# zhangmozhe/Deep-Exemplar-based-Video-Colorization

Hardware: AMD Instinct MI355X
Metric: colorized frames/sec/GPU at 216x384; correlation HBM GB/s vs roofline (higher is better)
Workload: dtype f32

## Files before the change

deep-exemplar-based-video-colorization_amd/csrc/conv_mfma.hip:

```cpp
#include "conv_kernel.h"
#include "conv_sk_kernel.h"
#include <algorithm>

#include "conv_wino_kernel.h"

static int virt_dim(int S, int up, int sub) {
    if (up == 2) return S * 2;
    if (sub == 2) return (S + 1) / 2;
    return S;
}

extern "C" int dvc_conv2d_out_hw(const DvcConvDesc* d, int32_t* OH, int32_t* OW) {
    DVC_REQUIRE(d, "dvc_conv2d_out_hw: null descriptor");
    int VH = virt_dim(d->H, d->in_up, d->in_sub), VW = virt_dim(d->W, d->in_up, d->in_sub);
    int ext = d->dil * (d->ksize - 1) + 1;
    *OH = (VH + 2 * d->pad - ext) / d->stride + 1;
    *OW = (VW + 2 * d->pad - ext) / d->stride + 1;
    return 0;
}

static int pick_tw(int OW) {
    int best = 32, best_w = cdiv(OW, 32) * 32;
    for (int tw : {16, 8}) {
        int wpad = cdiv(OW, tw) * tw;
// ... 575 lines not shown
    s.m_cls = wino_magic((long)s.blk_y * s.blk_x);
    s.m_blkx = wino_magic(s.blk_x);
    s.m_split = wino_magic(s.k.split);
    return dim3((unsigned)(s.gx * s.gy * s.gz));
}

static int wino_reduce(const DvcConvDesc* d, const ConvWinoArgs& s, int NB, int OH, int OW, const float* bias,
                       const float* act_slope_ptr, hipStream_t st) {
    const ConvKArgs& a = s.k;
    const long OHW = (long)OH * OW, per_img = (long)d->Cout * OHW;
    if (a.split > 1 && s.pool) {
        const long windows = (long)d->Cout * ((OH + 1) / 2) * ((OW + 1) / 2);
        hipLaunchKernelGGL(conv_splitk_reduce_pool_kernel, dim3((unsigned)((windows + 255) / 256), NB), dim3(256), 0, st, a.part,
                           a.split, (long)NB * per_img, d->Cout, OH, OW, bias, d->act, d->act_slope, act_slope_ptr, a.y, a.y_bs,
                           s.pool, s.pool_bs);
        DVC_CHECK_LAUNCH("dvc_conv2d_winograd_pool(split-K reduce)");
    } else if (a.split > 1 && !(d->flags & DVC_CONV_DEFER_REDUCE)) {
        const bool v4 = (OHW % 4 == 0) && ((reinterpret_cast<uintptr_t>(a.part) & 15) == 0) && (((long)NB * per_img) % 4 == 0);
        if (v4)
            hipLaunchKernelGGL(conv_splitk_reduce_kernel<4>, dim3((unsigned)((per_img / 4 + 255) / 256), NB), dim3(256), 0, st,
                               a.part, a.split, (long)NB * per_img, d->Cout, OHW, bias, a.res, a.res_bs, d->act,
                               d->act_slope, act_slope_ptr, a.y, a.y_bs);
        else
            hipLaunchKernelGGL(conv_splitk_reduce_kernel<1>, dim3((unsigned)((per_img + 255) / 256), NB), dim3(256), 0, st,
                               a.part, a.split, (long)NB * per_img, d->Cout, OHW, bias, a.res, a.res_bs, d->act,
                               d->act_slope, act_slope_ptr, a.y, a.y_bs);
        DVC_CHECK_LAUNCH("dvc_conv2d_winograd(split-K reduce)");
    }
    return 0;
}

static int wino_run(const DvcConvDesc* d, const DvcConvDesc* d2, const float* x, const float* x2, const float* u_packed,
                    const float* bias, const float* act_slope_ptr, const float* residual, float* y, void* workspace,
                    size_t workspace_bytes, dvcStream stream, float* pool = nullptr, long pool_batch_stride = 0) {
    ConvWinoArgs s;
    int best_m = -1, best_tr = 1, group = 0;
    if (int rc = wino_setup(d, d2, x, x2, u_packed, bias, act_slope_ptr, residual, y, workspace, workspace_bytes, pool,
                            pool_batch_stride, s, &best_m, &best_tr, &group))
        return rc;
    ConvKArgs& a = s.k;
    int32_t OH, OW;
    dvc_conv2d_out_hw(d, &OH, &OW);
    hipStream_t st = (hipStream_t)stream;
    for (int n0 = 0; n0 < d->N; n0 += group) {
        const int NB = std::min(group, d->N - n0);
        a.N = NB;
        a.x = x + (long)n0 * a.x_bs;
        if (d2) s.x2 = x2 + (long)n0 * s.x2_bs;
        a.y = y ? y + (long)n0 * a.y_bs : nullptr;
        s.pool = pool ? pool + (long)n0 * s.pool_bs : nullptr;
        a.res = residual ? residual + (long)n0 * a.res_bs : nullptr;
        DVC_REQUIRE((long)s.gx * s.gy * NB * a.split < (1L << 31), "dvc_conv2d_winograd: grid too large");
        const dim3 grid = wino_finish_grid(s, NB);
        if (d2) conv_wino_launch_m1_dual(best_tr, grid, st, s);
        else if (best_m == 0) conv_wino_launch_m4(best_tr, grid, st, s);
        else if (best_m == 1) conv_wino_launch_m2(best_tr, grid, st, s);
        else if (best_m == 2) conv_wino_launch_m1(best_tr, grid, st, s);
        else conv_wino_launch_m0(best_tr, grid, st, s);
        DVC_CHECK_LAUNCH("dvc_conv2d_winograd");
        if (int rc = wino_reduce(d, s, NB, OH, OW, bias, act_slope_ptr, st)) return rc;
    }
    return 0;
}

extern "C" int dvc_conv2d_winograd_group(const DvcConvGroupItem* items, int32_t n_items, dvcStream stream) {
    DVC_REQUIRE(items && n_items >= 1 && n_items <= WINO_GROUP_MAX, "dvc_conv2d_winograd_group: 1..%d items", WINO_GROUP_MAX);
    hipStream_t st = (hipStream_t)stream;
    ConvWinoGroupArgs g;
    int OHs[WINO_GROUP_MAX], OWs[WINO_GROUP_MAX], order[WINO_GROUP_MAX];
    ConvWinoArgs tmp[WINO_GROUP_MAX];
    int trs[WINO_GROUP_MAX];
    bool together = n_items > 1;
    for (int i = 0; i < n_items; ++i) {
        const DvcConvGroupItem& it = items[i];
        DVC_REQUIRE(it.x && it.u_packed && it.y, "dvc_conv2d_winograd_group: null argument in item %d", i);
        for (int j = 0; j < i; ++j) DVC_REQUIRE(it.y != items[j].y, "dvc_conv2d_winograd_group: items %d and %d share an output", j, i);
        int m = -1, grp = 0;
        if (int rc = wino_setup(&it.d, nullptr, it.x, nullptr, it.u_packed, it.bias, it.act_slope_ptr, it.residual, it.y, it.workspace,
                                it.workspace_bytes, nullptr, 0, tmp[i], &m, &trs[i], &grp))
            return rc;
        int32_t oh, ow;
        dvc_conv2d_out_hw(&it.d, &oh, &ow);
        OHs[i] = oh; OWs[i] = ow;
        if (m != 2 || grp < it.d.N) together = false;
        for (int j = 0; j < i; ++j)
            DVC_REQUIRE(!(tmp[i].k.split > 1 && tmp[j].k.split > 1 && tmp[i].k.part == tmp[j].k.part),
                        "dvc_conv2d_winograd_group: the split items %d and %d share a workspace", j, i);
        order[i] = i;
    }
    if (!together) {
        for (int i = 0; i < n_items; ++i) {
            const DvcConvGroupItem& it = items[i];
            if (int rc = wino_run(&it.d, nullptr, it.x, nullptr, it.u_packed, it.bias, it.act_slope_ptr, it.residual, it.y, it.workspace,
                                  it.workspace_bytes, stream))
                return rc;
        }
        return 0;
    }
    std::sort(order, order + n_items, [&](int a, int b) {
        return tmp[a].k.chunks_per_split != tmp[b].k.chunks_per_split ? tmp[a].k.chunks_per_split > tmp[b].k.chunks_per_split : a < b;
    });
    g.n = n_items;
    g.per_xcd[0] = 0;
    for (int k = 0; k < WINO_GROUP_MAX; ++k) {
        const int i = order[k < n_items ? k : n_items - 1];
        g.item[k] = tmp[i];
        g.tr[k] = trs[i];
// ... 95 lines not shown
```

deep-exemplar-based-video-colorization_amd/csrc/conv_wino_kernel.h:

```cpp
#pragma once
#include <type_traits>

#include "conv_kernel.h"

typedef float f32x4 __attribute__((ext_vector_type(4)));
typedef float f32x2 __attribute__((ext_vector_type(2)));

struct ConvWinoArgs {
    ConvKArgs k;
    int ss;
    int blk_y, blk_x;
    int gx, gy, gz;
    unsigned m_gx, m_gxy, m_cls, m_blkx, m_split;
    const float* x2;
    long x2_bs;
    int cinA, H2, W2, VH2, VW2, in_up2, in_sub2;
    float* pool;
    long pool_bs;
};
__host__ __device__ __forceinline__ unsigned wino_magic(long d) {
    return d > 1 ? (unsigned)(((1ULL << 32) + (unsigned long long)d - 1) / (unsigned long long)d) : 0u;
}
__device__ __forceinline__ int wino_div(int n, unsigned magic) { return magic ? (int)__umulhi((unsigned)n, magic) : n; }

__host__ __device__ constexpr int wino_pitch(int tr) { return tr == 1 ? 66 : tr == 2 ? 48 : tr == 4 ? 24 : 12; }

#define WINO_A10(p) "a" #p "0", "a" #p "1", "a" #p "2", "a" #p "3", "a" #p "4", "a" #p "5", "a" #p "6", "a" #p "7", "a" #p "8", "a" #p "9"
#define WINO_AGPRS                                                                                                     \
    WINO_A10(), WINO_A10(1), WINO_A10(2), WINO_A10(3), WINO_A10(4), WINO_A10(5), WINO_A10(6), WINO_A10(7), WINO_A10(8), \
        WINO_A10(9), WINO_A10(10), WINO_A10(11), "a120", "a121", "a122", "a123", "a124", "a125", "a126", "a127"
#define WINO_MFMA(K, A, B)                                                                \
    asm volatile("s_nop 1\n\tv_mfma_f32_32x32x2_f32 a[%2:%3], %0, %1, a[%2:%3]"            \
                 :                                                                         \
                 : "v"(A), "v"(B), "i"((K) * 16), "i"((K) * 16 + 15)                       \
                 : WINO_AGPRS)
#define WINO_PK_ADD(D, A, B) asm volatile("v_pk_add_f32 %0, %1, %2" : "=v"(D) : "v"(A), "v"(B))
#define WINO_PK_SUB(D, A, B) asm volatile("v_pk_add_f32 %0, %1, %2 neg_lo:[0,1] neg_hi:[0,1]" : "=v"(D) : "v"(A), "v"(B))
#define WINO_PK_MID(D, A, B) \
    asm volatile("v_pk_add_f32 %0, %1, %2 op_sel:[0,1] op_sel_hi:[0,1] neg_hi:[0,1]" : "=v"(D) : "v"(A), "v"(B))

#define WINO_LOADS(D, U, XA, UA, UOFS)                                                                                 \
    asm volatile("ds_read2_b64 %0, %5 offset0:%7 offset1:%8\n\t"                                                        \
                 "ds_read2_b64 %1, %5 offset0:%9 offset1:%10\n\t"                                                       \
                 "ds_read2_b64 %2, %5 offset0:%11 offset1:%12\n\t"                                                      \
                 "ds_read_b128 %3, %6 offset:%13\n\t"                                                                   \
                 "ds_read_b128 %4, %6 offset:%14"                                                                       \
                 : "=&v"(D[0]), "=&v"(D[1]), "=&v"(D[2]), "=&v"(U[0]), "=&v"(U[1])                                      \
                 : "v"(XA), "v"(UA), "i"(0 * (PITCH / 2)), "i"(0 * (PITCH / 2) + 1), "i"(1 * (PITCH / 2)),              \
                   "i"(1 * (PITCH / 2) + 1), "i"(2 * (PITCH / 2)), "i"(2 * (PITCH / 2) + 1), "i"((UOFS) + 0),           \
                   "i"((UOFS) + 512)                                                                                    \
                 : "memory")
#define WINO_WAIT_LOADS(D, U)                                                                 \
    asm volatile("s_waitcnt lgkmcnt(0)"                                                        \
                 : "+v"(D[0]), "+v"(D[1]), "+v"(D[2]), "+v"(U[0]), "+v"(U[1])                  \
                 :                                                                             \
                 : "memory")

#define WINO_S_ADD(D, A, B) asm volatile("v_add_f32 %0, %1, %2" : "=v"(D) : "v"(A), "v"(B))
#define WINO_S_SUB(D, A, B) asm volatile("v_sub_f32 %0, %1, %2" : "=v"(D) : "v"(A), "v"(B))

__device__ __forceinline__ int wino_stored_offset(int VH, int VW, int W, int in_up, int in_sub, int pad_mode, int vy, int vx) {
    int sy = map_virtual(vy, VH, pad_mode);
    int sx = map_virtual(vx, VW, pad_mode);
    if (sy < 0 || sx < 0) return -1;
    if (in_up == 2) {
        sy >>= 1;
        sx >>= 1;
    } else if (in_sub == 2) {
        sy <<= 1;
        sx <<= 1;
    }
    return sy * W + sx;
}

#define WINO_NBUF 3
__host__ __device__ constexpr int wino_xs_floats(int wm, int wn, int tr, int kc) {
    return ((kc * (2 * tr * wn + 2) * wino_pitch(tr) + 128 * wm * wn - 1) / (128 * wm * wn)) * (128 * wm * wn);
}
__host__ __device__ constexpr int wino_us_floats(int wm, int kc) { return wm * kc * 128 * 4; }

template <int WM, int WN, int TR, int KC, int VAR = 0, bool DUAL = false, class SA = ConvWinoArgs>
__device__ __forceinline__ void conv_wino_body(const SA& s, const int wlog, float* const xsb, float* const usb) {
#if defined(__HIP_DEVICE_COMPILE__)
    const auto& a = s.k;
    constexpr int NPAIR = WM * WN;
    constexpr int NT = 128 * NPAIR;
    constexpr int TC = 32 / TR;
    constexpr int PR = 2 * TR * WN + 2;
    constexpr int PC = 2 * TC + 2;
    constexpr int PITCH = wino_pitch(TR);
    constexpr int plane = PR * PITCH;
    constexpr int EPT = (KC * plane + NT - 1) / NT;
    constexpr int C_XS = EPT * NT;
    static_assert(C_XS == wino_xs_floats(WM, WN, TR, KC), "LDS size helper out of step");
    constexpr int UQ = WM * KC * 128;
    static_assert(UQ * 4 == wino_us_floats(WM, KC), "LDS size helper out of step");
    static_assert(UQ % NT == 0, "whole staging instructions");
    static_assert(PITCH >= PC && PITCH % 2 == 0 && plane % 2 == 0 && KC % 4 == 0, "aligned patch rows, even K-steps per chunk");
    static_assert(2 * (PITCH / 2) + 1 < 256, "ds_read2_b64 offsets are 8 bits");
    constexpr int WPT = UQ / NT;
    constexpr int NI = EPT + WPT;
    static_assert(2 * NI < 64, "vmcnt is 6 bits");
    constexpr int KS = KC / 2;
    constexpr int NBUF = WINO_NBUF;
    constexpr int OOB = (int)0x80000000;
    static_assert(NBUF * UQ * 4 >= 2 * NPAIR * 32 * 64, "the output exchange fits in the filter buffers");

    const int tid = threadIdx.x;
    const int lane = tid & 63, wave = __builtin_amdgcn_readfirstlane(tid >> 6);
    const int l31 = lane & 31, hi = lane >> 5;
    const int ph = wave / NPAIR, pair = wave % NPAIR;
    const int wm = pair / WN, wn = pair % WN;
    const int tr = l31 / TC, tc = l31 % TC;
    const int ss = s.ss;
    const int bz = wino_div(wlog, s.m_gxy), r_xy = wlog - bz * (s.gx * s.gy);
    const int by = wino_div(r_xy, s.m_gx), bx = r_xy - by * s.gx;
    const int per_cls = s.blk_y * s.blk_x;
    const int cls = wino_div(bx, s.m_cls), brem = bx - cls * per_cls;
    const int py = ss == 2 ? cls >> 1 : 0, px = ss == 2 ? cls & 1 : 0;
    const int tyb = wino_div(brem, s.m_blkx);
    const int ty0 = tyb * (TR * WN), tx0 = (brem - tyb * s.blk_x) * TC;
    const int b0 = by * WM;
    const int n = wino_div(bz, s.m_split), ksplit = bz - n * a.split;
    const int HWi = a.H * a.W;

    const int nchunks_all = a.Cin / KC;
    const int c_begin = ksplit * a.chunks_per_split;
    const int c_end = min(nchunks_all, c_begin + a.chunks_per_split);

    int gofs[EPT], wrel[WPT];
#pragma unroll
    for (int i = 0; i < WPT; ++i) {
        const int q = tid + i * NT;
        wrel[i] = ((q / (KC * 128)) * a.Cin * 128 + q % (KC * 128)) * 16;
    }
    __amdgpu_buffer_rsrc_t rs_w =
        __builtin_amdgcn_make_buffer_rsrc((void*)(a.w + (long)b0 * a.Cin * 512), 0, WM * a.Cin * 2048, 0x00020000);
    auto issue_w = [&](int c, int buf) {
        const int sw = c * KC * 2048;
        float* us = usb + buf * (UQ * 4);
#pragma unroll
        for (int i = 0; i < WPT; ++i)
            __builtin_amdgcn_raw_ptr_buffer_load_lds(rs_w, (CONV_AS3 void*)(us + (i * NT + wave * 64) * 4), 16, wrel[i], sw, 0, 0);
    };
    issue_w(c_begin, 0);
    asm volatile(".set wino_i, 0\n\t.rept 128\n\tv_accvgpr_write_b32 a[wino_i], 0\n\t.set wino_i, wino_i + 1\n\t.endr" ::: WINO_AGPRS);
#pragma unroll
    for (int t = 0; t < EPT; ++t) {
        const int e = tid + t * NT;
        const int c = e / plane, rem = e - c * plane;
        const int iy = rem / PITCH, ix = rem - iy * PITCH;
        int g = -1;
        if (e < KC * plane && ix < PC) {
            const int o = stored_offset(a, ss * (2 * ty0 - 1 + iy) + py, ss * (2 * tx0 - 1 + ix) + px);
            if (o >= 0) g = c * HWi + o;
        }
        gofs[t] = g >= 0 ? g * 4 : OOB;
    }
    const int cinA = DUAL ? s.cinA : a.Cin;
// ... 53 lines not shown
        else if (c_begin + 1 < c_end) asm volatile("s_waitcnt vmcnt(%0)" ::"n"(NI) : "memory");
        else asm volatile("s_waitcnt vmcnt(0)" ::: "memory");
    }
    __builtin_amdgcn_s_barrier();

    const float slope = a.act_slope_ptr ? *a.act_slope_ptr : a.act_slope;
    const long OHW = (long)a.OH * a.OW;
    const bool partial = a.split > 1;
    float* yb = partial ? a.part + ((long)ksplit * a.N + n) * a.Cout * OHW : a.y + (long)n * a.y_bs;
    const float* rb = (!partial && a.res) ? a.res + (long)n * a.res_bs : nullptr;

    auto run = [&](auto PHC) {
        constexpr int PH = decltype(PHC)::value;
        f32x4 D[2][3], U[2][2];
        f32x2 V03[2][2], V12[2][2];
        auto lo = [](const f32x4& v) { return __builtin_shufflevector(v, v, 0, 1); };
        auto hh = [](const f32x4& v) { return __builtin_shufflevector(v, v, 2, 3); };
        auto transform_a = [&](const f32x4 (&d)[3], f32x2 (&tl)[2], f32x2 (&th)[2]) {
            if (VAR == 1) {
                if (PH == 0) {
                    WINO_S_SUB(tl[0].x, d[0].x, d[2].x); WINO_S_SUB(tl[0].y, d[0].y, d[2].y);
                    WINO_S_SUB(th[0].x, d[0].z, d[2].z); WINO_S_SUB(th[0].y, d[0].w, d[2].w);
                    WINO_S_ADD(tl[1].x, d[1].x, d[2].x); WINO_S_ADD(tl[1].y, d[1].y, d[2].y);
                    WINO_S_ADD(th[1].x, d[1].z, d[2].z); WINO_S_ADD(th[1].y, d[1].w, d[2].w);
                } else {
                    WINO_S_SUB(tl[0].x, d[1].x, d[0].x); WINO_S_SUB(tl[0].y, d[1].y, d[0].y);
                    WINO_S_SUB(th[0].x, d[1].z, d[0].z); WINO_S_SUB(th[0].y, d[1].w, d[0].w);
                    WINO_S_SUB(tl[1].x, d[0].x, d[2].x); WINO_S_SUB(tl[1].y, d[0].y, d[2].y);
                    WINO_S_SUB(th[1].x, d[0].z, d[2].z); WINO_S_SUB(th[1].y, d[0].w, d[2].w);
                }
                return;
            }
            if (PH == 0) {
                WINO_PK_SUB(tl[0], lo(d[0]), lo(d[2]));
                WINO_PK_SUB(th[0], hh(d[0]), hh(d[2]));
                WINO_PK_ADD(tl[1], lo(d[1]), lo(d[2]));
                WINO_PK_ADD(th[1], hh(d[1]), hh(d[2]));
            } else {
                WINO_PK_SUB(tl[0], lo(d[1]), lo(d[0]));
                WINO_PK_SUB(th[0], hh(d[1]), hh(d[0]));
                WINO_PK_SUB(tl[1], lo(d[0]), lo(d[2]));
                WINO_PK_SUB(th[1], hh(d[0]), hh(d[2]));
            }
        };
        auto transform_b = [&](const f32x2& tl, const f32x2& th, f32x2& v03, f32x2& v12) {
            if (VAR == 1) {
                WINO_S_SUB(v03.x, tl.x, th.x); WINO_S_SUB(v03.y, tl.y, th.y);
                WINO_S_ADD(v12.x, th.x, tl.y); WINO_S_SUB(v12.y, th.x, tl.y);
                return;
            }
            WINO_PK_SUB(v03, tl, th);
            WINO_PK_MID(v12, th, tl);
        };
        {
            f32x2 tl[2], th[2];
            WINO_LOADS(D[0], U[0], xlane, ulane, 0);
            WINO_WAIT_LOADS(D[0], U[0]);
            transform_a(D[0], tl, th);
            transform_b(tl[0], th[0], V03[0][0], V12[0][0]);
            transform_b(tl[1], th[1], V03[0][1], V12[0][1]);
        }

        int buf = 0;
        for (int c = c_begin; c < c_end; ++c) {
            const unsigned xb = xlane + buf * (C_XS * 4), ub = ulane + buf * (UQ * 16);
            const int nbuf = buf == NBUF - 1 ? 0 : buf + 1;
            const unsigned xbn = xlane + nbuf * (C_XS * 4), ubn = ulane + nbuf * (UQ * 16);
            const bool more = c + 1 < c_end;
#pragma unroll
            for (int ks = 0; ks < KS; ++ks) {
                const int cs = ks & 1, ns = cs ^ 1;
                const bool last = ks == KS - 1;
                f32x2 tl[2], th[2];
                WINO_MFMA(0, U[cs][0].x, V03[cs][0].x);
                if (!last) {
                    WINO_LOADS(D[ns], U[ns], xb + (ks + 1) * (2 * plane * 4), ub, (ks + 1) * 4096);
                } else if (BRANCH_FREE) {
                    asm volatile("s_waitcnt vmcnt(%0)" ::"n"(NI) : "memory");
                    __builtin_amdgcn_s_barrier();
                    issue(min(c + 3, c_end - 1), buf);
                    WINO_LOADS(D[ns], U[ns], xbn, ubn, 0);
                } else if (more) {
                    if (c + 2 < c_end) asm volatile("s_waitcnt vmcnt(%0)" ::"n"(NI) : "memory");
                    else asm volatile("s_waitcnt vmcnt(0)" ::: "memory");
                    __builtin_amdgcn_s_barrier();
                    if (c + 3 < c_end) issue(c + 3, buf);
                    WINO_LOADS(D[ns], U[ns], xbn, ubn, 0);
                }
                __builtin_amdgcn_sched_barrier(0);
                WINO_MFMA(1, U[cs][0].y, V12[cs][0].x);
                WINO_MFMA(2, U[cs][0].z, V12[cs][0].y);
                WINO_MFMA(3, U[cs][0].w, V03[cs][0].y);
                WINO_WAIT_LOADS(D[ns], U[ns]);
                __builtin_amdgcn_sched_barrier(0);
                transform_a(D[ns], tl, th);
                __builtin_amdgcn_sched_barrier(0);
                WINO_MFMA(4, U[cs][1].x, V03[cs][1].x);
                transform_b(tl[0], th[0], V03[ns][0], V12[ns][0]);
                __builtin_amdgcn_sched_barrier(0);
                WINO_MFMA(5, U[cs][1].y, V12[cs][1].x);
                transform_b(tl[1], th[1], V03[ns][1], V12[ns][1]);
                __builtin_amdgcn_sched_barrier(0);
                WINO_MFMA(6, U[cs][1].z, V12[cs][1].y);
                WINO_MFMA(7, U[cs][1].w, V03[cs][1].y);
                __builtin_amdgcn_sched_barrier(0);
            }
            buf = nbuf;
        }
        asm volatile("s_waitcnt vmcnt(0)" ::: "memory");
        __builtin_amdgcn_s_barrier();

        float* ex = usb;
        asm volatile("s_nop 15\n\ts_nop 7" ::: WINO_AGPRS);
        auto partial_out = [&](auto RC, float (&o)[4]) {
            constexpr int r = decltype(RC)::value;
            float m[8];
#pragma unroll
            for (int k = 0; k < 8; ++k) asm volatile("v_accvgpr_read_b32 %0, a[%1]" : "=v"(m[k]) : "i"(k * 16 + r) : WINO_AGPRS);
            float s0[4], s1[4];
#pragma unroll
            for (int j = 0; j < 4; ++j) {
                if (PH == 0) {
                    s0[j] = m[j] + m[4 + j];
                    s1[j] = m[4 + j];
                } else {
                    s0[j] = m[j];
                    s1[j] = -m[j] - m[4 + j];
                }
            }
            o[0] = s0[0] + s0[1] + s0[2];
            o[1] = s0[1] - s0[2] - s0[3];
            o[2] = s1[0] + s1[1] + s1[2];
            o[3] = s1[1] - s1[2] - s1[3];
        };
        auto for8 = [&](auto f) {
            f(std::integral_constant<int, 0>{}); f(std::integral_constant<int, 1>{}); f(std::integral_constant<int, 2>{});
            f(std::integral_constant<int, 3>{}); f(std::integral_constant<int, 4>{}); f(std::integral_constant<int, 5>{});
            f(std::integral_constant<int, 6>{}); f(std::integral_constant<int, 7>{});
        };
        {
            float* mine = ex + (wave * 32) * 64 + lane;
            for8([&](auto IC) {
                constexpr int i = decltype(IC)::value;
                float o[4];
                partial_out(std::integral_constant<int, 8 * (1 - PH) + i>{}, o);
#pragma unroll
                for (int q = 0; q < 4; ++q) mine[(i * 4 + q) * 64] = o[q];
            });
        }
        __syncthreads();
        const float* theirs = ex + ((PH == 0 ? wave + NPAIR : wave - NPAIR) * 32) * 64 + lane;
        const int u0 = 2 * (ty0 + wn * TR + tr), x0 = 2 * (tx0 + tc);
        const int oy0 = ss * u0 + py, oy1 = ss * (u0 + 1) + py;
        const int ox0 = ss * x0 + px, ox1 = ss * (x0 + 1) + px;
        const bool okx0 = ox0 < a.OW, okx1 = ox1 < a.OW;
        const bool pairst = ss == 1 && okx1 && (a.OW & 1) == 0;
        const bool pool_here = !partial && s.pool;
        float* pb = pool_here ? s.pool + (long)n * s.pool_bs : nullptr;
        const long PHW = (long)(a.OH >> 1) * (a.OW >> 1);
        for8([&](auto IC) {
            constexpr int i = decltype(IC)::value;
            constexpr int r = 8 * PH + i;
            float o[4];
            partial_out(std::integral_constant<int, r>{}, o);
#pragma unroll
            for (int q = 0; q < 4; ++q) {
                const float t = theirs[(i * 4 + q) * 64];
                o[q] = PH == 0 ? o[q] + t : t + o[q];
            }
            const int co = (b0 + wm) * 32 + (r & 3) + 8 * (r >> 2) + 4 * hi;
            const float bias = (!partial && a.bias) ? a.bias[co] : 0.f;
            float pooled = 0.f;
#pragma unroll
            for (int p = 0; p < 2; ++p) {
                const int oy = p ? oy1 : oy0;
                if (oy >= a.OH) continue;
                const long row = (long)co * OHW + (long)oy * a.OW;
                float v0 = o[2 * p] + bias, v1 = o[2 * p + 1] + bias;
                if (rb) {
                    if (okx0) v0 += rb[row + ox0];
                    if (okx1) v1 += rb[row + ox1];
                }
                if (!partial) {
                    v0 = apply_act(v0, a.act, slope);
                    v1 = apply_act(v1, a.act, slope);
                }
                if (pool_here) {
                    const float m = fmaxf(v0, v1);
                    pooled = p ? fmaxf(pooled, m) : m;
                    if (p && okx1) pb[(long)co * PHW + (long)(oy0 >> 1) * (a.OW >> 1) + (ox0 >> 1)] = pooled;
                    if (!a.y) continue;
                }
                if (pairst && VAR == 2) {
                    union { float2 f; unsigned long long u; } cv;
                    cv.f = make_float2(v0, v1);
                    __hip_atomic_store(reinterpret_cast<unsigned long long*>(yb + row + ox0), cv.u, __ATOMIC_RELAXED, __HIP_MEMORY_SCOPE_AGENT);
                } else if (pairst) {
                    *reinterpret_cast<float2*>(yb + row + ox0) = make_float2(v0, v1);
                } else {
                    if (okx0) yb[row + ox0] = v0;
                    if (okx1) yb[row + ox1] = v1;
                }
            }
        });
    };
    if (ph) run(std::integral_constant<int, 1>{});
    else run(std::integral_constant<int, 0>{});
#endif
}

template <int WM, int WN, int TR, int KC, int VAR = 0, bool DUAL = false>
__global__ __launch_bounds__(128 * WM * WN) __attribute__((amdgpu_waves_per_eu(2, 2))) void conv_wino_kernel(ConvWinoArgs s) {
    __shared__ __attribute__((aligned(16))) float xsb[WINO_NBUF * wino_xs_floats(WM, WN, TR, KC)];
    __shared__ __attribute__((aligned(16))) float usb[WINO_NBUF * wino_us_floats(WM, KC)];
    const int G = s.gx * s.gy * s.gz;
    const int xq = G / 8, xr = G % 8, xcd = blockIdx.x % 8, xi = blockIdx.x / 8;
    const int wlog = (xcd < xr ? xcd * (xq + 1) : xr * (xq + 1) + (xcd - xr) * xq) + xi;
    conv_wino_body<WM, WN, TR, KC, VAR, DUAL>(s, wlog, xsb, usb);
}

#define WINO_GROUP_MAX 4
struct ConvWinoGroupArgs {
    ConvWinoArgs item[WINO_GROUP_MAX];
    int per_xcd[WINO_GROUP_MAX + 1];
    int tr[WINO_GROUP_MAX];
    int n;
};
typedef __attribute__((address_space(4))) ConvWinoArgs ConvWinoArgsK;
template <int WM, int WN, int KC>
__global__ __launch_bounds__(128 * WM * WN) __attribute__((amdgpu_waves_per_eu(2, 2))) void conv_wino_group_kernel(ConvWinoGroupArgs g) {
    constexpr int XS = wino_xs_floats(WM, WN, 1, KC) > wino_xs_floats(WM, WN, 8, KC) ? wino_xs_floats(WM, WN, 1, KC) : wino_xs_floats(WM, WN, 8, KC);
    static_assert(XS >= wino_xs_floats(WM, WN, 2, KC) && XS >= wino_xs_floats(WM, WN, 4, KC), "largest patch buffer");
#if defined(__HIP_DEVICE_COMPILE__)
    __shared__ __attribute__((aligned(16))) float xsb[WINO_NBUF * XS];
    __shared__ __attribute__((aligned(16))) float usb[WINO_NBUF * wino_us_floats(WM, KC)];
    const int xcd = blockIdx.x % 8, xi = blockIdx.x / 8;
    int it = 0, base = 0, q = g.per_xcd[1], tr = g.tr[0];
#pragma unroll
    for (int i = 1; i < WINO_GROUP_MAX; ++i)
        if (i < g.n && xi >= g.per_xcd[i]) {
            it = i;
            base = g.per_xcd[i];
            q = g.per_xcd[i + 1] - g.per_xcd[i];
            tr = g.tr[i];
        }
    const int wlog = xcd * q + (xi - base);
    static_assert(__builtin_offsetof(ConvWinoGroupArgs, item) == 0, "item table at the start of the argument block");
    const ConvWinoArgsK& s = ((const ConvWinoArgsK*)__builtin_amdgcn_kernarg_segment_ptr())[it];
    if (wlog >= s.gx * s.gy * s.gz) return;
    switch (tr) {
        case 1: conv_wino_body<WM, WN, 1, KC, 0, false, ConvWinoArgsK>(s, wlog, xsb, usb); break;
        case 2: conv_wino_body<WM, WN, 2, KC, 0, false, ConvWinoArgsK>(s, wlog, xsb, usb); break;
        case 4: conv_wino_body<WM, WN, 4, KC, 0, false, ConvWinoArgsK>(s, wlog, xsb, usb); break;
        default: conv_wino_body<WM, WN, 8, KC, 0, false, ConvWinoArgsK>(s, wlog, xsb, usb); break;
    }
#endif
}

template <int WM, int WN, int KC>
static void conv_wino_launch_shape(int tr, dim3 grid, hipStream_t st, const ConvWinoArgs& s) {
    constexpr int NT = 128 * WM * WN;
#ifdef DVC_DEBUG
    if (s.k.dbg & 8) {
        switch (tr) {
            case 1: hipLaunchKernelGGL((conv_wino_kernel<WM, WN, 1, KC, 3>), grid, dim3(NT), 0, st, s); break;
            case 2: hipLaunchKernelGGL((conv_wino_kernel<WM, WN, 2, KC, 3>), grid, dim3(NT), 0, st, s); break;
            case 4: hipLaunchKernelGGL((conv_wino_kernel<WM, WN, 4, KC, 3>), grid, dim3(NT), 0, st, s); break;
            default: hipLaunchKernelGGL((conv_wino_kernel<WM, WN, 8, KC, 3>), grid, dim3(NT), 0, st, s); break;
        }
        return;
    }
    if (s.k.dbg & 32) {
        switch (tr) {
            case 1: hipLaunchKernelGGL((conv_wino_kernel<WM, WN, 1, KC, 2>), grid, dim3(NT), 0, st, s); break;
            case 2: hipLaunchKernelGGL((conv_wino_kernel<WM, WN, 2, KC, 2>), grid, dim3(NT), 0, st, s); break;
            case 4: hipLaunchKernelGGL((conv_wino_kernel<WM, WN, 4, KC, 2>), grid, dim3(NT), 0, st, s); break;
            default: hipLaunchKernelGGL((conv_wino_kernel<WM, WN, 8, KC, 2>), grid, dim3(NT), 0, st, s); break;
        }
        return;
    }
    if (s.k.dbg & 16) {
        switch (tr) {
            case 1: hipLaunchKernelGGL((conv_wino_kernel<WM, WN, 1, KC, 1>), grid, dim3(NT), 0, st, s); break;
            case 2: hipLaunchKernelGGL((conv_wino_kernel<WM, WN, 2, KC, 1>), grid, dim3(NT), 0, st, s); break;
            case 4: hipLaunchKernelGGL((conv_wino_kernel<WM, WN, 4, KC, 1>), grid, dim3(NT), 0, st, s); break;
            default: hipLaunchKernelGGL((conv_wino_kernel<WM, WN, 8, KC, 1>), grid, dim3(NT), 0, st, s); break;
        }
        return;
    }
#endif
    const unsigned dyn = (kDvcDebug && (s.k.dbg & 512)) ? 36u * 1024u : 0u;
    switch (tr) {
        case 1: hipLaunchKernelGGL((conv_wino_kernel<WM, WN, 1, KC>), grid, dim3(NT), dyn, st, s); break;
        case 2: hipLaunchKernelGGL((conv_wino_kernel<WM, WN, 2, KC>), grid, dim3(NT), dyn, st, s); break;
        case 4: hipLaunchKernelGGL((conv_wino_kernel<WM, WN, 4, KC>), grid, dim3(NT), dyn, st, s); break;
        default: hipLaunchKernelGGL((conv_wino_kernel<WM, WN, 8, KC>), grid, dim3(NT), dyn, st, s); break;
    }
}

template <int WM, int WN, int KC>
static void conv_wino_launch_shape_dual(int tr, dim3 grid, hipStream_t st, const ConvWinoArgs& s) {
    constexpr int NT = 128 * WM * WN;
    switch (tr) {
        case 1: hipLaunchKernelGGL((conv_wino_kernel<WM, WN, 1, KC, 0, true>), grid, dim3(NT), 0, st, s); break;
        case 2: hipLaunchKernelGGL((conv_wino_kernel<WM, WN, 2, KC, 0, true>), grid, dim3(NT), 0, st, s); break;
        case 4: hipLaunchKernelGGL((conv_wino_kernel<WM, WN, 4, KC, 0, true>), grid, dim3(NT), 0, st, s); break;
        default: hipLaunchKernelGGL((conv_wino_kernel<WM, WN, 8, KC, 0, true>), grid, dim3(NT), 0, st, s); break;
    }
}

void conv_wino_launch_m1_dual(int tr, dim3 grid, hipStream_t st, const ConvWinoArgs& s);
void conv_wino_launch_m4(int tr, dim3 grid, hipStream_t st, const ConvWinoArgs& s);
void conv_wino_launch_m2(int tr, dim3 grid, hipStream_t st, const ConvWinoArgs& s);
void conv_wino_launch_m1(int tr, dim3 grid, hipStream_t st, const ConvWinoArgs& s);
void conv_wino_launch_m0(int tr, dim3 grid, hipStream_t st, const ConvWinoArgs& s);
void conv_wino_launch_group_m1(dim3 grid, hipStream_t st, const ConvWinoGroupArgs& g);
```

deep-exemplar-based-video-colorization_amd/csrc/conv_wino_m1.hip:

```cpp
#include "conv_wino_kernel.h"

void conv_wino_launch_m1(int tr, dim3 grid, hipStream_t st, const ConvWinoArgs& s) {
    conv_wino_launch_shape<2, 1, 4>(tr, grid, st, s);
}

void conv_wino_launch_m1_dual(int tr, dim3 grid, hipStream_t st, const ConvWinoArgs& s) {
    conv_wino_launch_shape_dual<2, 1, 4>(tr, grid, st, s);
}
```

deep-exemplar-based-video-colorization_amd/dvc_amd/ops.py:

```python
import ctypes
import os as _os
import sys
from typing import NamedTuple

import torch

from . import _lib
from ._lib import DvcConvDesc, DvcConvGroupItem, DvcInstNormItem

ACT_NONE, ACT_RELU, ACT_PRELU, ACT_LEAKY, ACT_TANH128 = 0, 1, 2, 3, 4
PAD_ZERO, PAD_REFLECT = 0, 1
EPS64 = sys.float_info.epsilon


def _p(t):
    return None if t is None else ctypes.c_void_p(t.data_ptr())


def _pv(t):
    return None if t is None else t.data_ptr()


_raw_stream = getattr(torch._C, "_cuda_getCurrentRawStream", None)
_raw_device = getattr(torch._C, "_cuda_getDevice", None)
# ... 140 lines not shown


def set_autotune(flag=True):
    global _autotune
    _autotune = bool(flag)
    if _autotune:
        _load_tuned()


def conv_algo():
    return _conv_algo


def set_conv_algo(algo):
    global _conv_algo
    if algo not in ("auto", "speed", "direct", "winograd"):
        raise ValueError("conv algo must be 'auto', 'speed', 'direct' or 'winograd'")
    _conv_algo = algo


def exemplar_memo_enabled():
    return _exemplar_memo != "off"


def exemplar_memo_mode():
    return _exemplar_memo


def set_exemplar_memo(flag=True):
    global _exemplar_memo
    _exemplar_memo = "verify" if flag == "verify" else ("on" if flag else "off")


_direct_layers = None


def direct_layers():
    if _direct_layers is not None:
        return _direct_layers
    if DEFAULT_DIRECT_LAYERS is not None:
        return DEFAULT_DIRECT_LAYERS
    from . import arch
    return arch.DIRECT_LAYERS


def set_direct_layers(names=None):
    global _direct_layers
    _direct_layers = None if names is None else frozenset(names)


DEFER_REDUCE = 1
BATCH_PLAN = 2
GRAY_INPUT = 4


class batch_plan:

    def __init__(self, on=True):
        self.on = bool(on)

    def __enter__(self):
        global _batch_plan
        self.prev, _batch_plan = _batch_plan, self.on
        return self

    def __exit__(self, *exc):
        global _batch_plan
        _batch_plan = self.prev


def batch_plan_enabled():
    return _batch_plan


def _plan_flags(N):
    return BATCH_PLAN if (_batch_plan and N > 1) else 0


_tuned = {}

_cache_path = _os.environ.get("DVC_AUTOTUNE_CACHE")
_cache_loaded = False


def _load_tuned():
    global _cache_loaded
    if _cache_loaded or not _cache_path:
        return
    _cache_loaded = True
    try:
        import json
        with open(_cache_path) as f:
            for k, v in json.load(f).items():
                _tuned[tuple(json.loads(k))] = tuple(v)
    except (OSError, ValueError):
        pass


def _save_tuned():
    if not _cache_path:
        return
    import json
    tmp = _cache_path + ".tmp%d" % _os.getpid()
    with open(tmp, "w") as f:
        json.dump({json.dumps(list(k)): list(v) for k, v in _tuned.items()}, f)
    _os.replace(tmp, _cache_path)
# ... 269 lines not shown
        conv_record.append(_record_conv(d, affine=False, in_prelu=False, residual=residual is not None, algo="winograd"))
    ws = _workspace(x.device, CONV_WORKSPACE_BYTES, ws_tag)
    generation = _bump_generation(ws)
    S = 1
    if defer_reduce and residual is None and _may_defer(act, OH, OW):
        S, ipl = _winograd_split(lib, d, ws.numel())
        if S > 1 and ipl >= N and S * N * Cout * OH * OW * 4 <= ws.numel():
            d.flags |= DEFER_REDUCE
        else:
            S = 1
    if S == 1 and out is None:
        out = torch.empty((N, Cout, OH, OW), device=x.device, dtype=torch.float32)
    rc = lib.dvc_conv2d_winograd(ctypes.byref(d), _p(x), _p(u_packed), _p(bias), _p(act_slope_t), _p(residual),
                                 _p(out) if out is not None else ctypes.c_void_p(ws.data_ptr()),
                                 ctypes.c_void_p(ws.data_ptr()), ws.numel(), _stream())
    _lib.check(rc, "dvc_conv2d_winograd")
    if S > 1:
        return ConvPartials(ws, S, (N, Cout, OH, OW), bias, act, float(act_slope), act_slope_t, generation, x.device)
    return out


def conv2d_winograd_pool(x, u_packed, bias, *, act=ACT_NONE, act_slope=0.0, act_slope_t=None, pad_mode=PAD_ZERO, want_full=True):
    lib = _lib.load()
    _need_all(x=x, u_packed=u_packed, bias=bias, act_slope=act_slope_t)
    N, Cin, H, W = x.shape
    assert u_packed.dim() == 5 and u_packed.shape[1] == Cin and tuple(u_packed.shape[2:]) == (4, 32, 4), u_packed.shape
    Cout = u_packed.shape[0] * 32
    d = _conv_desc(N, Cin, H, W, Cout, pad_mode=pad_mode, act=act, act_slope=act_slope, flags=_plan_flags(N))
    if conv_record is not None:
        conv_record.append(_record_conv(d, affine=False, in_prelu=False, residual=False, algo="winograd"))
    ws = _workspace(x.device, CONV_WORKSPACE_BYTES, "conv")
    _bump_generation(ws)
    full = torch.empty((N, Cout, H, W), device=x.device, dtype=torch.float32) if want_full else None
    pooled = torch.empty((N, Cout, H // 2, W // 2), device=x.device, dtype=torch.float32)
    _lib.check(lib.dvc_conv2d_winograd_pool(ctypes.byref(d), _p(x), _p(u_packed), _p(bias), _p(act_slope_t), _p(full), _p(pooled), 0,
                                            ctypes.c_void_p(ws.data_ptr()), ws.numel(), _stream()),
               "dvc_conv2d_winograd_pool")
    return full, pooled


def conv2d_winograd_dual(xA, xB, u_cat, bias, *, dil=1, pad_mode=PAD_ZERO, in_upA=1, in_upB=1, act=ACT_NONE, act_slope=0.0,
                         act_slope_t=None):
    lib = _lib.load()
    _need_all(xA=xA, xB=xB, u_cat=u_cat, bias=bias, act_slope=act_slope_t)
    N, CA, HA, WA = xA.shape
    NB, CB, HB, WB = xB.shape
    assert N == NB and u_cat.dim() == 5 and u_cat.shape[1] == CA + CB and tuple(u_cat.shape[2:]) == (4, 32, 4), (xA.shape, xB.shape, u_cat.shape)
    Cout = u_cat.shape[0] * 32
    OH, OW = conv_out_hw(HA, WA, 3, 1, dil, dil, in_upA, 1)
    if (OH, OW) != conv_out_hw(HB, WB, 3, 1, dil, dil, in_upB, 1):
        raise RuntimeError(f"dvc_amd: conv2d_winograd_dual: the two inputs' virtual sizes differ ({HA * in_upA} x {WA * in_upA} vs "
                           f"{HB * in_upB} x {WB * in_upB})")
    common = dict(dil=dil, pad_mode=pad_mode, act=act, act_slope=act_slope)
    dA = _conv_desc(N, CA, HA, WA, Cout, in_up=in_upA, flags=_plan_flags(N), **common)
    dB = _conv_desc(N, CB, HB, WB, Cout, in_up=in_upB, **common)
    if conv_record is not None:
        conv_record.append(_record_conv(_conv_desc(N, CA + CB, OH, OW, Cout, **common), affine=False, in_prelu=False,
                                        residual=False, algo="winograd-dual"))
    ws = _workspace(xA.device, CONV_WORKSPACE_BYTES, "conv")
    _bump_generation(ws)
    out = torch.empty((N, Cout, OH, OW), device=xA.device, dtype=torch.float32)
    _lib.check(lib.dvc_conv2d_winograd_dual(ctypes.byref(dA), ctypes.byref(dB), _p(xA), _p(xB), _p(u_cat), _p(bias), _p(act_slope_t),
                                            _p(out), ctypes.c_void_p(ws.data_ptr()), ws.numel(), _stream()),
               "dvc_conv2d_winograd_dual")
    return out


def conv3x3(x, weight, packs, bias, *, dil=1, pad_mode=PAD_ZERO, in_up=1, in_sub=1, act=ACT_NONE, act_slope=0.0,
            act_slope_t=None, residual=None, out=None, out_batch_stride=0, defer_reduce=False, layer=None, ws_tag="conv"):
    N, Cin, H, W = x.shape
    Cout = weight.shape[0]
    if layer_record is not None:
        record_layer(layer, Cin, Cout, H, W, dil=dil, in_up=in_up, in_sub=in_sub,
                     eligible=winograd_eligible(Cin, Cout, 3, 1, dil, dil)
                     and _wino_rule(N, Cin, Cout, *conv_out_hw(H, W, 3, 1, dil, dil, in_up, in_sub), dil))
    if winograd_selected(N, Cin, H, W, Cout, dil=dil, pad=dil, in_up=in_up, in_sub=in_sub, layer=layer):
        return conv2d_winograd(x, packs("winograd"), bias, dil=dil, pad_mode=pad_mode, in_up=in_up, in_sub=in_sub,
                               act=act, act_slope=act_slope, act_slope_t=act_slope_t, residual=residual, out=out,
                               out_batch_stride=out_batch_stride, defer_reduce=defer_reduce and _fuse_reduce, ws_tag=ws_tag)
    if _ws_conv and residual is None and ws_eligible(Cin, Cout, dil, pad_mode, in_up, in_sub, act):
        return conv2d_ws(x, packs("ws"), bias, Cout, act=act, act_slope=act_slope, act_slope_t=act_slope_t, out=out,
                         out_batch_stride=out_batch_stride)
    return conv2d(x, packs("direct"), bias, dil=dil, pad=dil, pad_mode=pad_mode, in_up=in_up, in_sub=in_sub, act=act,
                  act_slope=act_slope, act_slope_t=act_slope_t, residual=residual, out=out,
                  out_batch_stride=out_batch_stride, tune=not (_conv_algo == "auto" and layer is not None and layer in direct_layers()))


def _item_is_winograd(it):
    N, Cin, H, W = it["x"].shape
    dil = it.get("dil", 1)
    return winograd_selected(N, Cin, H, W, it["weight"].shape[0], dil=dil, pad=dil, in_up=it.get("in_up", 1),
                             in_sub=it.get("in_sub", 1), layer=it.get("layer"))


def conv3x3_group(items):
    def single(it, i=0):
        kw = {k: v for k, v in it.items() if k not in ("x", "weight", "packs", "bias")}
        own = i > 0 or not all(_item_is_winograd(o) for o in items[1:])
        return conv3x3(it["x"], it["weight"], it["packs"], it["bias"], ws_tag=f"conv.g{i}" if own else "conv", **kw)

    n = len(items)
    if not (_group_heads and 2 <= n <= 4 and all(it.get("out") is None and it.get("residual") is None and _item_is_winograd(it)
                                                 for it in items)):
        return [single(it, i) for i, it in enumerate(items)]
    lib = _lib.load()
    dev = items[0]["x"].device
    ws = _workspace(dev, CONV_WORKSPACE_BYTES, "conv")
# ... 631 lines not shown
```

include/dvc_hip.h:

```cpp
#ifndef DVC_HIP_H
#define DVC_HIP_H

#include <stddef.h>
#include <stdint.h>

#ifdef __cplusplus
extern "C" {
#endif

#pragma GCC visibility push(default)

typedef void* dvcStream;

#define DVC_ABI_VERSION 20

int dvc_abi_version(void);
const char* dvc_last_error(void);

enum { DVC_ACT_NONE = 0, DVC_ACT_RELU = 1, DVC_ACT_PRELU = 2, DVC_ACT_LEAKY = 3, DVC_ACT_TANH128 = 4 };
enum { DVC_PAD_ZERO = 0, DVC_PAD_REFLECT = 1 };

typedef struct DvcConvDesc {
    int32_t N, Cin, H, W;
    int32_t Cout;
    int32_t ksize;
    int32_t stride;
    int32_t dil;
    int32_t pad;
    int32_t pad_mode;
    int32_t in_up;
    int32_t in_sub;
    int32_t act;
    float   act_slope;
    int32_t in_prelu;
    int32_t cfg;
    int32_t split_k;
    int64_t x_batch_stride;
    int64_t y_batch_stride;
    int64_t res_batch_stride;
    int32_t flags;
    int64_t w_batch_stride;
} DvcConvDesc;
#define DVC_CONV_DEFER_REDUCE 1
#define DVC_CONV_BATCH_PLAN 2
#define DVC_CONV_GRAY_INPUT 4

int dvc_conv2d_out_hw(const DvcConvDesc* d, int32_t* OH, int32_t* OW);

int dvc_conv2d(const DvcConvDesc* d,
               const float* x, const float* w_packed, const float* bias ,
               const float* in_scale , const float* in_shift ,
               const float* in_slope_ptr ,
               const float* act_slope_ptr ,
               const float* residual , float* y,
               void* workspace , size_t workspace_bytes,
               dvcStream stream);

size_t dvc_winograd_weight_floats(int32_t Cout, int32_t Cin);
int dvc_winograd_pack_weight(const float* w, int32_t Cout, int32_t Cin, float* u_packed, dvcStream stream);
int dvc_conv2d_winograd_split(const DvcConvDesc* d, size_t workspace_bytes, int32_t* split, int32_t* images_per_launch);
int dvc_conv2d_winograd(const DvcConvDesc* d, const float* x, const float* u_packed,
                        const float* bias , const float* act_slope_ptr ,
                        const float* residual , float* y,
                        void* workspace , size_t workspace_bytes, dvcStream stream);
int dvc_conv2d_winograd_pool(const DvcConvDesc* d, const float* x, const float* u_packed, const float* bias ,
                             const float* act_slope_ptr , float* y , float* y_pool,
                             int64_t pool_batch_stride, void* workspace , size_t workspace_bytes, dvcStream stream);
int dvc_conv2d_winograd_dual(const DvcConvDesc* dA, const DvcConvDesc* dB, const float* xA, const float* xB,
                             const float* u_packed_cat, const float* bias ,
                             const float* act_slope_ptr , float* y,
                             void* workspace , size_t workspace_bytes, dvcStream stream);

int dvc_conv2d_ws_eligible(const DvcConvDesc* d);
int dvc_conv2d_ws_pack_weight(const float* w, int32_t Cout, int32_t Cin, float* u_packed, dvcStream stream);
int dvc_conv2d_ws(const DvcConvDesc* d, const float* x, const float* u_packed, const float* bias ,
                  const float* act_slope_ptr , float* y, dvcStream stream);

typedef struct DvcConvGroupItem {
    DvcConvDesc d;
    const float* x;
    const float* u_packed;
    const float* bias;
    const float* act_slope_ptr;
    const float* residual;
    float* y;
    void* workspace;
    size_t workspace_bytes;
} DvcConvGroupItem;
int dvc_conv2d_winograd_group(const DvcConvGroupItem* items, int32_t n_items, dvcStream stream);

int dvc_conv1x1_small(const float* x, const float* w, const float* bias, int32_t N, int32_t Cin,
                      int32_t HW, int32_t Cout, int32_t act, float* y, dvcStream stream);

int dvc_instnorm_stats(const float* x, int32_t N, int32_t C, int32_t HW, int64_t x_batch_stride,
                       float eps, const float* chan_scale, float* scale, float* shift,
                       dvcStream stream);

int dvc_affine_act(const float* x, const float* scale, const float* shift, const float* residual,
// ... 165 lines not shown
```

Measured before the change: 432.6.

## Skip redundant Winograd MFMAs for nearest-upsampled inputs in dual conv

Adds an UPSKIP variant of the dual-input Winograd kernel. For an input that is 2x nearest-upsampled, adjacent transformed columns are duplicates, so some input-transform terms are zero or redundant. The variant skips two of the eight MFMAs per step and half the LDS loads on the odd phase, using a reduced transform. It is on by default through an env flag and a descriptor flag. The cost is more template instantiations, a more complex phase-dependent schedule, and a transition fixup between the A and B channel ranges that could be fragile.

```diff
diff --git a/deep-exemplar-based-video-colorization_amd/csrc/conv_mfma.hip b/deep-exemplar-based-video-colorization_amd/csrc/conv_mfma.hip
--- a/deep-exemplar-based-video-colorization_amd/csrc/conv_mfma.hip
+++ b/deep-exemplar-based-video-colorization_amd/csrc/conv_mfma.hip
@@ -651,7 +651,8 @@
         a.res = residual ? residual + (long)n0 * a.res_bs : nullptr;
         DVC_REQUIRE((long)s.gx * s.gy * NB * a.split < (1L << 31), "dvc_conv2d_winograd: grid too large");
         const dim3 grid = wino_finish_grid(s, NB);
-        if (d2) conv_wino_launch_m1_dual(best_tr, grid, st, s);
+        const bool upskip = d2 && s.ss == 1 && !(d->flags & DVC_CONV_NO_UPSKIP) && (a.in_up == 2 || s.in_up2 == 2);
+        if (d2) conv_wino_launch_m1_dual(best_tr, grid, st, s, upskip);
         else if (best_m == 0) conv_wino_launch_m4(best_tr, grid, st, s);
         else if (best_m == 1) conv_wino_launch_m2(best_tr, grid, st, s);
         else if (best_m == 2) conv_wino_launch_m1(best_tr, grid, st, s);
diff --git a/deep-exemplar-based-video-colorization_amd/csrc/conv_wino_kernel.h b/deep-exemplar-based-video-colorization_amd/csrc/conv_wino_kernel.h
--- a/deep-exemplar-based-video-colorization_amd/csrc/conv_wino_kernel.h
+++ b/deep-exemplar-based-video-colorization_amd/csrc/conv_wino_kernel.h
@@ -56,6 +56,16 @@
                  :                                                                             \
                  : "memory")
 
+#define WINO_LOADS_UP1(D, U, XA, UA, UOFS)                                                                             \
+    asm volatile("ds_read2_b64 %0, %3 offset0:%5 offset1:%6\n\t"                                                        \
+                 "ds_read2_b64 %1, %3 offset0:%7 offset1:%8\n\t"                                                        \
+                 "ds_read_b128 %2, %4 offset:%9"                                                                        \
+                 : "=&v"(D[0]), "=&v"(D[2]), "=&v"(U[1])                                                                \
+                 : "v"(XA), "v"(UA), "i"(0 * (PITCH / 2)), "i"(0 * (PITCH / 2) + 1), "i"(2 * (PITCH / 2)),              \
+                   "i"(2 * (PITCH / 2) + 1), "i"((UOFS) + 512)                                                          \
+                 : "memory")
+#define WINO_WAIT_LOADS_UP1(D, U) asm volatile("s_waitcnt lgkmcnt(0)" : "+v"(D[0]), "+v"(D[2]), "+v"(U[1]) : : "memory")
+
 #define WINO_S_ADD(D, A, B) asm volatile("v_add_f32 %0, %1, %2" : "=v"(D) : "v"(A), "v"(B))
 #define WINO_S_SUB(D, A, B) asm volatile("v_sub_f32 %0, %1, %2" : "=v"(D) : "v"(A), "v"(B))
 
@@ -79,7 +89,7 @@
 }
 __host__ __device__ constexpr int wino_us_floats(int wm, int kc) { return wm * kc * 128 * 4; }
 
-template <int WM, int WN, int TR, int KC, int VAR = 0, bool DUAL = false, class SA = ConvWinoArgs>
+template <int WM, int WN, int TR, int KC, int VAR = 0, bool DUAL = false, class SA = ConvWinoArgs, bool UPSKIP = false>
 __device__ __forceinline__ void conv_wino_body(const SA& s, const int wlog, float* const xsb, float* const usb) {
 #if defined(__HIP_DEVICE_COMPILE__)
     const auto& a = s.k;
@@ -105,6 +115,7 @@
     constexpr int NBUF = WINO_NBUF;
     constexpr int OOB = (int)0x80000000;
     static_assert(NBUF * UQ * 4 >= 2 * NPAIR * 32 * 64, "the output exchange fits in the filter buffers");
+    static_assert(!UPSKIP || (DUAL && VAR == 0), "UPSKIP is built for the two-input kernels only");
 
     const int tid = threadIdx.x;
     const int lane = tid & 63, wave = __builtin_amdgcn_readfirstlane(tid >> 6);
@@ -264,6 +275,10 @@
             WINO_PK_SUB(v03, tl, th);
             WINO_PK_MID(v12, th, tl);
         };
+        auto transform_b_up = [&](const f32x2& tl, const f32x2& th, f32x2& v03, f32x2& v12) {
+            WINO_PK_SUB(v03, tl, th);
+            WINO_S_ADD(v12.x, th.x, tl.y);
+        };
         {
             f32x2 tl[2], th[2];
             WINO_LOADS(D[0], U[0], xlane, ulane, 0);
@@ -274,6 +289,7 @@
         }
 
         int buf = 0;
+        if constexpr (!UPSKIP) {
         for (int c = c_begin; c < c_end; ++c) {
             const unsigned xb = xlane + buf * (C_XS * 4), ub = ulane + buf * (UQ * 16);
             const int nbuf = buf == NBUF - 1 ? 0 : buf + 1;
@@ -319,6 +335,101 @@
             }
             buf = nbuf;
         }
+        } else {
+        auto chunk = [&](auto UPC, const int c) {
+            constexpr bool UP = decltype(UPC)::value;
+            const unsigned xb = xlane + buf * (C_XS * 4), ub = ulane + buf * (UQ * 16);
+            const int nbuf = buf == NBUF - 1 ? 0 : buf + 1;
+            const unsigned xbn = xlane + nbuf * (C_XS * 4), ubn = ulane + nbuf * (UQ * 16);
+            const bool more = c + 1 < c_end;
+#pragma unroll
+            for (int ks = 0; ks < KS; ++ks) {
+                const int cs = ks & 1, ns = cs ^ 1;
+                const bool last = ks == KS - 1;
+                f32x2 tl[2], th[2];
+                if (UP && PH == 1) WINO_MFMA(4, U[cs][1].x, V03[cs][1].x);
+                else WINO_MFMA(0, U[cs][0].x, V03[cs][0].x);
+                if (!last) {
+                    if (UP && PH == 1) WINO_LOADS_UP1(D[ns], U[ns], xb + (ks + 1) * (2 * plane * 4), ub, (ks + 1) * 4096);
+                    else WINO_LOADS(D[ns], U[ns], xb + (ks + 1) * (2 * plane * 4), ub, (ks + 1) * 4096);
+                } else if (BRANCH_FREE) {
+                    asm volatile("s_waitcnt vmcnt(%0)" ::"n"(NI) : "memory");
+                    __builtin_amdgcn_s_barrier();
+                    issue(min(c + 3, c_end - 1), buf);
+                    WINO_LOADS(D[ns], U[ns], xbn, ubn, 0);
+                } else if (more) {
+                    if (c + 2 < c_end) asm volatile("s_waitcnt vmcnt(%0)" ::"n"(NI) : "memory");
+                    else asm volatile("s_waitcnt vmcnt(0)" ::: "memory");
+                    __builtin_amdgcn_s_barrier();
+                    if (c + 3 < c_end) issue(c + 3, buf);
+                    WINO_LOADS(D[ns], U[ns], xbn, ubn, 0);
+                }
+                __builtin_amdgcn_sched_barrier(0);
+                if (UP) {
+                    if (PH == 0) {
+                        WINO_MFMA(1, U[cs][0].y, V12[cs][0].x);
+                        WINO_MFMA(3, U[cs][0].w, V03[cs][0].y);
+                        WINO_WAIT_LOADS(D[ns], U[ns]);
+                        __builtin_amdgcn_sched_barrier(0);
+                        transform_a(D[ns], tl, th);
+                        __builtin_amdgcn_sched_barrier(0);
+                        WINO_MFMA(4, U[cs][1].x, V03[cs][1].x);
+                        transform_b_up(tl[0], th[0], V03[ns][0], V12[ns][0]);
+                        __builtin_amdgcn_sched_barrier(0);
+                        WINO_MFMA(5, U[cs][1].y, V12[cs][1].x);
+                        transform_b_up(tl[1], th[1], V03[ns][1], V12[ns][1]);
+                        __builtin_amdgcn_sched_barrier(0);
+                        WINO_MFMA(7, U[cs][1].w, V03[cs][1].y);
+                    } else {
+                        WINO_MFMA(5, U[cs][1].y, V12[cs][1].x);
+                        WINO_MFMA(7, U[cs][1].w, V03[cs][1].y);
+                        if (!last) WINO_WAIT_LOADS_UP1(D[ns], U[ns]);
+                        else WINO_WAIT_LOADS(D[ns], U[ns]);
+                        __builtin_amdgcn_sched_barrier(0);
+                        WINO_PK_SUB(tl[1], lo(D[ns][0]), lo(D[ns][2]));
+                        WINO_PK_SUB(th[1], hh(D[ns][0]), hh(D[ns][2]));
+                        transform_b_up(tl[1], th[1], V03[ns][1], V12[ns][1]);
+                    }
+                    __builtin_amdgcn_sched_barrier(0);
+                    continue;
+                }
+                WINO_MFMA(1, U[cs][0].y, V12[cs][0].x);
+                WINO_MFMA(2, U[cs][0].z, V12[cs][0].y);
+                WINO_MFMA(3, U[cs][0].w, V03[cs][0].y);
+                WINO_WAIT_LOADS(D[ns], U[ns]);
+                __builtin_amdgcn_sched_barrier(0);
+                transform_a(D[ns], tl, th);
+                __builtin_amdgcn_sched_barrier(0);
+                WINO_MFMA(4, U[cs][1].x, V03[cs][1].x);
+                transform_b(tl[0], th[0], V03[ns][0], V12[ns][0]);
+                __builtin_amdgcn_sched_barrier(0);
+                WINO_MFMA(5, U[cs][1].y, V12[cs][1].x);
+                transform_b(tl[1], th[1], V03[ns][1], V12[ns][1]);
+                __builtin_amdgcn_sched_barrier(0);
+                WINO_MFMA(6, U[cs][1].z, V12[cs][1].y);
+                WINO_MFMA(7, U[cs][1].w, V03[cs][1].y);
+                __builtin_amdgcn_sched_barrier(0);
+            }
+            buf = nbuf;
+        };
+        auto kloop = [&](auto UPC, const int c0, const int c1) {
+            for (int c = c0; c < c1; ++c) chunk(UPC, c);
+        };
+        {
+            const int c_mid = min(max(nchA, c_begin), c_end);
+            const bool upA = a.in_up == 2 && ss == 1, upB = s.in_up2 == 2 && ss == 1;
+            if (upA) kloop(std::true_type{}, c_begin, c_mid);
+            else kloop(std::false_type{}, c_begin, c_mid);
+            if (upA && !upB && c_begin < c_mid && c_mid < c_end) {
+                f32x2 tl[2], th[2];
+                transform_a(D[0], tl, th);
+                transform_b(tl[0], th[0], V03[0][0], V12[0][0]);
+                transform_b(tl[1], th[1], V03[0][1], V12[0][1]);
+            }
+            if (upB) kloop(std::true_type{}, c_mid, c_end);
+            else kloop(std::false_type{}, c_mid, c_end);
+        }
+        }
         asm volatile("s_waitcnt vmcnt(0)" ::: "memory");
         __builtin_amdgcn_s_barrier();
 
@@ -421,14 +532,14 @@
 #endif
 }
 
-template <int WM, int WN, int TR, int KC, int VAR = 0, bool DUAL = false>
+template <int WM, int WN, int TR, int KC, int VAR = 0, bool DUAL = false, bool UPSKIP = false>
 __global__ __launch_bounds__(128 * WM * WN) __attribute__((amdgpu_waves_per_eu(2, 2))) void conv_wino_kernel(ConvWinoArgs s) {
     __shared__ __attribute__((aligned(16))) float xsb[WINO_NBUF * wino_xs_floats(WM, WN, TR, KC)];
     __shared__ __attribute__((aligned(16))) float usb[WINO_NBUF * wino_us_floats(WM, KC)];
     const int G = s.gx * s.gy * s.gz;
     const int xq = G / 8, xr = G % 8, xcd = blockIdx.x % 8, xi = blockIdx.x / 8;
     const int wlog = (xcd < xr ? xcd * (xq + 1) : xr * (xq + 1) + (xcd - xr) * xq) + xi;
-    conv_wino_body<WM, WN, TR, KC, VAR, DUAL>(s, wlog, xsb, usb);
+    conv_wino_body<WM, WN, TR, KC, VAR, DUAL, ConvWinoArgs, UPSKIP>(s, wlog, xsb, usb);
 }
 
 #define WINO_GROUP_MAX 4
@@ -511,8 +622,17 @@
 }
 
 template <int WM, int WN, int KC>
-static void conv_wino_launch_shape_dual(int tr, dim3 grid, hipStream_t st, const ConvWinoArgs& s) {
+static void conv_wino_launch_shape_dual(int tr, dim3 grid, hipStream_t st, const ConvWinoArgs& s, bool upskip) {
     constexpr int NT = 128 * WM * WN;
+    if (upskip) {
+        switch (tr) {
+            case 1: hipLaunchKernelGGL((conv_wino_kernel<WM, WN, 1, KC, 0, true, true>), grid, dim3(NT), 0, st, s); break;
+            case 2: hipLaunchKernelGGL((conv_wino_kernel<WM, WN, 2, KC, 0, true, true>), grid, dim3(NT), 0, st, s); break;
+            case 4: hipLaunchKernelGGL((conv_wino_kernel<WM, WN, 4, KC, 0, true, true>), grid, dim3(NT), 0, st, s); break;
+            default: hipLaunchKernelGGL((conv_wino_kernel<WM, WN, 8, KC, 0, true, true>), grid, dim3(NT), 0, st, s); break;
+        }
+        return;
+    }
     switch (tr) {
         case 1: hipLaunchKernelGGL((conv_wino_kernel<WM, WN, 1, KC, 0, true>), grid, dim3(NT), 0, st, s); break;
         case 2: hipLaunchKernelGGL((conv_wino_kernel<WM, WN, 2, KC, 0, true>), grid, dim3(NT), 0, st, s); break;
@@ -521,7 +641,7 @@
     }
 }
 
-void conv_wino_launch_m1_dual(int tr, dim3 grid, hipStream_t st, const ConvWinoArgs& s);
+void conv_wino_launch_m1_dual(int tr, dim3 grid, hipStream_t st, const ConvWinoArgs& s, bool upskip);
 void conv_wino_launch_m4(int tr, dim3 grid, hipStream_t st, const ConvWinoArgs& s);
 void conv_wino_launch_m2(int tr, dim3 grid, hipStream_t st, const ConvWinoArgs& s);
 void conv_wino_launch_m1(int tr, dim3 grid, hipStream_t st, const ConvWinoArgs& s);
diff --git a/deep-exemplar-based-video-colorization_amd/csrc/conv_wino_m1.hip b/deep-exemplar-based-video-colorization_amd/csrc/conv_wino_m1.hip
--- a/deep-exemplar-based-video-colorization_amd/csrc/conv_wino_m1.hip
+++ b/deep-exemplar-based-video-colorization_amd/csrc/conv_wino_m1.hip
@@ -4,6 +4,6 @@
     conv_wino_launch_shape<2, 1, 4>(tr, grid, st, s);
 }
 
-void conv_wino_launch_m1_dual(int tr, dim3 grid, hipStream_t st, const ConvWinoArgs& s) {
-    conv_wino_launch_shape_dual<2, 1, 4>(tr, grid, st, s);
+void conv_wino_launch_m1_dual(int tr, dim3 grid, hipStream_t st, const ConvWinoArgs& s, bool upskip) {
+    conv_wino_launch_shape_dual<2, 1, 4>(tr, grid, st, s, upskip);
 }
diff --git a/deep-exemplar-based-video-colorization_amd/dvc_amd/ops.py b/deep-exemplar-based-video-colorization_amd/dvc_amd/ops.py
--- a/deep-exemplar-based-video-colorization_amd/dvc_amd/ops.py
+++ b/deep-exemplar-based-video-colorization_amd/dvc_amd/ops.py
@@ -216,6 +216,22 @@
 DEFER_REDUCE = 1
 BATCH_PLAN = 2
 GRAY_INPUT = 4
+NO_UPSKIP = 8
+
+
+_wino_upskip = _on_unless_0(_os.environ.get("DVC_WINO_UPSKIP", "1"))
+
+
+def wino_upskip_enabled():
+    return _wino_upskip
+
+
+def set_wino_upskip(flag=True):
+    global _wino_upskip
+    if bool(flag) != _wino_upskip:
+        _wino_upskip = bool(flag)
+        from . import nets
+        nets.invalidate_weight_caches()
 
 
 class batch_plan:
@@ -591,7 +607,7 @@
         raise RuntimeError(f"dvc_amd: conv2d_winograd_dual: the two inputs' virtual sizes differ ({HA * in_upA} x {WA * in_upA} vs "
                            f"{HB * in_upB} x {WB * in_upB})")
     common = dict(dil=dil, pad_mode=pad_mode, act=act, act_slope=act_slope)
-    dA = _conv_desc(N, CA, HA, WA, Cout, in_up=in_upA, flags=_plan_flags(N), **common)
+    dA = _conv_desc(N, CA, HA, WA, Cout, in_up=in_upA, flags=_plan_flags(N) | (0 if _wino_upskip else NO_UPSKIP), **common)
     dB = _conv_desc(N, CB, HB, WB, Cout, in_up=in_upB, **common)
     if conv_record is not None:
         conv_record.append(_record_conv(_conv_desc(N, CA + CB, OH, OW, Cout, **common), affine=False, in_prelu=False,
diff --git a/include/dvc_hip.h b/include/dvc_hip.h
--- a/include/dvc_hip.h
+++ b/include/dvc_hip.h
@@ -44,6 +44,7 @@
 #define DVC_CONV_DEFER_REDUCE 1
 #define DVC_CONV_BATCH_PLAN 2
 #define DVC_CONV_GRAY_INPUT 4
+#define DVC_CONV_NO_UPSKIP 8
 
 int dvc_conv2d_out_hw(const DvcConvDesc* d, int32_t* OH, int32_t* OW);
 
```

After: 436.8 (median of 6 runs). Within noise of the previous version (+1.0%).
